# blackle/Megalania

Hardware: AMD Instinct MI355X
Metric: SA neighbour-cost evals/s (higher is better)
Workload: dtype u64

## Files before the change

megalania_amd/csrc/mgl_api.hip:

```cpp
#include "mgl_kernels.hip"
#include "mgl_kernels2.hip"
#include "mgl_kernels3.hip"
#include "mgl_kernels4.hip"
#include "mgl_kernels5.hip"
#include "mgl_pbuild.hip"
#include "mgl_index.hip"
#include "mgl_matchfinder.hip"
#include "mgl_optimal.hip"
#include "mgl_adaptive.hip"
#include "mgl_props.hip"
#include "../../include/megalania_hip.h"

#include <math.h>
#include <stdio.h>
#include <stdlib.h>
#include <string.h>
#include <string>
#include <vector>

static const uint16_t k_cost_table[2048] = {
#include "mgl_cost_table.inc"
};

#define MGL_MAX_INPUT 176000000ull
// ... 398 lines not shown
		HIPCHK(hipGetLastError());
		return MGL_OK;
	}
	if (zero_counts) HIPCHK(hipMemsetAsync(sa->d_counts, 0, 8 * sizeof(uint32_t), sa->stream));
	const uint32_t blocks2 = (K + sa->waves_per_block2 - 1) / sa->waves_per_block2;
	const bool split_now = sa->split_nbr && !sa->form_single;
	const uint32_t sim_lds_regular = ((((sa->ctx.L.total + 31u) >> 5) + 3u) & ~3u) * 4u + sa->chg_cap * 16u;
	if (split_now) {
		const uint32_t slices = nbr_slices(sa);
		HIPCHK(hipEventRecord(sa->ev_fork, sa->stream));
		if (slices >= 2) HIPCHK(hipStreamWaitEvent(sa->stream2, sa->ev_fork, 0));
		HIPCHK(hipStreamWaitEvent(sa->stream3, sa->ev_fork, 0));
		for (uint32_t h = 0; h < slices; h++) {
			const uint32_t j0 = (uint32_t)((uint64_t)K * h / slices), j1 = (uint32_t)((uint64_t)K * (h + 1) / slices);
			hipStream_t st = (h & 1u) ? sa->stream2 : sa->stream;
			hipLaunchKernelGGL((k_neighbours2<false, MGL_NBR_PICK>), dim3((j1 - j0 + sa->pick_waves - 1) / sa->pick_waves), dim3(64 * sa->pick_waves),
			                   (MGL_PICK_T_GLOBAL ? 0u : 4096u) + sa->pick_waves * sa->per_wave_pick, st, sa->ctx,
			                   sa->b2, sa->base.ctl, sa->cfg.seed, step_override, K, sa->nbr, sa->per_wave_pick, sa->d_todo, sa->d_counts,
			                   (unsigned long long*)nullptr, sa->big, sa->d_pickrec, j0, j1, sa->d_pickstate); NBR_TRACE("k_neighbours2<false, MGL_NBR_PICK>");
			hipLaunchKernelGGL((k_neighbours2<false, MGL_NBR_REST>), dim3(j1 - j0), dim3(64), sa->per_wave_rest, st, sa->ctx,
			                   sa->b2, sa->base.ctl, sa->cfg.seed, step_override, K, sa->nbr, sa->per_wave_rest, sa->d_todo, sa->d_counts,
			                   g_prof_big ? (unsigned long long*)nullptr : sa->d_prof, sa->big, sa->d_pickrec, j0, j1, sa->d_pickstate); NBR_TRACE("k_neighbours2<false, MGL_NBR_REST>");
			HIPCHK(hipEventRecord(sa->ev_rest[h], st));
		}
		HIPCHK(hipGetLastError());
		for (uint32_t h = 0; h < slices; h++) {
			const uint32_t j0 = (uint32_t)((uint64_t)K * h / slices), j1 = (uint32_t)((uint64_t)K * (h + 1) / slices);
			HIPCHK(hipStreamWaitEvent(sa->stream3, sa->ev_rest[h], 0));
			if (sa->time_sim_step >= 0 && h < 2) HIPCHK(hipEventRecord(sim_event(sa, 4 * (size_t)sa->time_sim_step + 2 * h), sa->stream3));
			if (sa->count_traffic)
				hipLaunchKernelGGL(k_sim<true>, dim3(j1 - j0), dim3(64 * sa->sim_waves), sim_lds_regular, sa->stream3, sa->ctx, sa->b2, sa->base.ctl,
				                   sa->nbr, sa->big, j0, j1, sa->d_todo3, sa->d_counts + 4, sa->d_traffic);
			else
				hipLaunchKernelGGL(k_sim<false>, dim3(j1 - j0), dim3(64 * sa->sim_waves), sim_lds_regular, sa->stream3, sa->ctx, sa->b2, sa->base.ctl,
// ... 323 lines not shown
		sa->snapshots = !(sa->cfg.flags & MGL_F_NO_SNAPSHOTS);
		if (sa->snapshots) {
			for (Base2* s : { &sa->snap_lit, &sa->snap_best }) {
				*s = b;
				s->slab = nullptr; s->onwalk = nullptr; s->sp0 = s->sp1 = s->sp2 = nullptr; s->sp_state = nullptr;
				s->ck_probs = nullptr; s->ch_off = s->ch_len = s->ch_cap = s->ch_pos = nullptr; s->ch_ev = nullptr;
				s->pool_top = nullptr;
				int rc = alloc_b2(*s, n, true, false, nullptr);
				if (rc) return rc;
			}
			HIPCHK(hipMalloc(&sa->d_snap_meta, sizeof(SnapMeta) * 2));
			HIPCHK(hipMemset(sa->d_snap_meta, 0, sizeof(SnapMeta) * 2));
			sa->d_best = sa->snap_best.slab;
		}
		if (sa->cfg.flags & MGL_F_PROFILE) {
			HIPCHK(hipMalloc(&sa->d_prof, sizeof(unsigned long long) * (32 + K)));
			HIPCHK(hipMemset(sa->d_prof, 0, sizeof(unsigned long long) * (32 + K)));
		}
		HIPCHK(hipMalloc(&sa->d_todo, sizeof(uint32_t) * (K + 1)));
		HIPCHK(hipMemset(sa->d_todo, 0, sizeof(uint32_t) * (K + 1)));
		sa->b2_bytes = bytes;
		sa->incremental_apply = getenv("MGL_NO_INCREMENTAL_APPLY") == nullptr;
		{
			ApplyBuf& ab = sa->ab;
			memset(&ab, 0, sizeof ab);
			sa->apply_blocks = 256;
			ab.scratch_cap = b.pool_cap + 256u;
			ab.span_cap = 1u << 22;
			ab.job_cap = 1u << 20;
			HIPCHK(hipMalloc(&ab.hdr, sizeof(uint32_t) * 16));
			HIPCHK(hipMemset(ab.hdr, 0, sizeof(uint32_t) * 16));
			HIPCHK(hipMalloc(&ab.ins_key, sizeof(uint16_t) * MGL_BATCH_ALLOC));
// ... 75 lines not shown
				const uint32_t tot = (160u * 1024u / bytes) * w;
				if (tot > best_total) { best_total = tot; best_w = w; }
			}
			(void)best_w;
			sa->waves_per_block2 = 1;
		}
		sa->nbr2_lds = 4096u + sa->waves_per_block2 * sa->per_wave2;
		sa->build_lds = 4096u + ckpt_elems * 2u + ckpt_elems * 8u;
		HIPCHK(hipMalloc(&sa->d_counts, sizeof(uint32_t) * 16));
		HIPCHK(hipMemset(sa->d_counts, 0, sizeof(uint32_t) * 16));
		HIPCHK(hipMalloc(&sa->d_todo3, sizeof(uint32_t) * (K + 1)));
		HIPCHK(hipMemset(sa->d_todo3, 0, sizeof(uint32_t) * (K + 1)));
		sa->big.todo_in = sa->d_todo; sa->big.todo_in_count = sa->d_counts; sa->big.spill_ctr = sa->d_counts + 2;
		HIPCHK(hipFuncSetAttribute((const void*)k_neighbours2<false, MGL_NBR_FULL>, hipFuncAttributeMaxDynamicSharedMemorySize, (int)sa->nbr2_lds));
		HIPCHK(hipFuncSetAttribute((const void*)k_neighbours2<false, MGL_NBR_PICK>, hipFuncAttributeMaxDynamicSharedMemorySize, 160 * 1024));
		HIPCHK(hipFuncSetAttribute((const void*)k_neighbours2<false, MGL_NBR_REST>, hipFuncAttributeMaxDynamicSharedMemorySize, (int)sa->nbr2_lds));
		HIPCHK(hipFuncSetAttribute((const void*)k_neighbours2<true, MGL_NBR_FULL>, hipFuncAttributeMaxDynamicSharedMemorySize, (int)(4096u + sa->per_wave2 + 12u * MGL_BIG_CAP + MGL_COOP_BYTES)));
		HIPCHK(hipMalloc(&sa->d_pickrec, sizeof(uint4) * K));
		HIPCHK(hipMalloc(&sa->d_pickstate, sizeof(uint4) * 2 * K));
		sa->split_nbr = getenv("MGL_NO_SPLIT") == nullptr;
		if (sa->split_nbr) {
			BigScratch& g = sa->big;
			HIPCHK(hipMalloc(&g.sim_hdr, sizeof(uint4) * (size_t)K));
			HIPCHK(hipMalloc(&g.sim_keys, sizeof(uint16_t) * 2u * sa->chg_cap * (size_t)K));
			HIPCHK(hipMalloc(&g.sim_pos, sizeof(uint32_t) * 2u * sa->chg_cap * (size_t)K));
			HIPCHK(hipMemset(g.sim_hdr, 0xFF, sizeof(uint4) * (size_t)K));
			if (getenv("MGL_NO_CONT") == nullptr) {
				HIPCHK(hipMalloc(&g.cont, sizeof(uint32_t) * MGL_CONT_WORDS * (size_t)g.slots));
				HIPCHK(hipMemset(g.cont, 0, sizeof(uint32_t) * MGL_CONT_WORDS * (size_t)g.slots));
			}
// ... 1208 lines not shown
	const Base2& b = sa->b2;
	const void* src = nullptr;
	size_t sz = 0;
	uint32_t top = 0;
	if (sa->incremental) HIPCHK(hipMemcpy(&top, b.pool_top, sizeof top, hipMemcpyDeviceToHost));
	switch (what) {
	case 0: src = b.ch_off; sz = sizeof(uint32_t) * sa->ctx.L.total; break;
	case 1: src = b.ch_len; sz = sizeof(uint32_t) * sa->ctx.L.total; break;
	case 2: src = b.ch_pos; sz = sizeof(uint32_t) * (size_t)top; break;
	case 3: src = b.ch_ev; sz = sizeof(uint16_t) * (size_t)top; break;
	case 4: src = b.onwalk; sz = sizeof(uint64_t) * b.nw0; break;
	case 5: src = b.sp0; sz = sizeof(uint64_t) * b.nw0; break;
	case 6: src = b.sp_state; sz = sizeof(uint32_t) * 8 * (size_t)sa->n; break;
	case 7: src = b.ck_probs; sz = sizeof(uint16_t) * (size_t)b.nck * b.ck_elems; break;
	case 8: src = b.ch_cap; sz = sizeof(uint32_t) * sa->ctx.L.total; break;
	case 9: src = sa->d_prof; sz = sa->d_prof ? sizeof(unsigned long long) * (32 + sa->cfg.neighbours_per_step) : 0; break;
	case 80: {
		const uint64_t v[3] = { sa->batch_accepts, sa->batch_fallbacks, sa->batch_early_giveups };
		*bytes = sizeof v;
		if (cap_bytes >= sizeof v) memcpy(out, v, sizeof v);
		return MGL_OK;
	}
	case 84: src = sa->lim.why; sz = sizeof(uint32_t); break;
	case 85: src = b.pool_top; sz = sizeof(uint32_t); break;
	case 83: src = b.ch_sb; sz = sizeof(uint32_t) * (size_t)b.ck_elems * b.sb_stride; break;
	case 81: src = sa->batch.hdr; sz = sizeof(uint32_t) * 16; break;
	case 82: src = sa->batch.acc; sz = sizeof(long long) * 4; break;
	case 10: src = sa->d_counts + 8; sz = sizeof(uint32_t) * 4; break;
	case 14: src = sa->ab.hdr; sz = sa->ab.hdr ? sizeof(uint32_t) * 16 : 0; break;
	case 16: src = sa->base.ctl; sz = sizeof(Control); break;
	case 15: src = sa->d_pickrec; sz = sa->d_pickrec ? sizeof(uint4) * sa->cfg.neighbours_per_step : 0; break;
// ... 76 lines not shown
```

megalania_amd/csrc/mgl_kernels.hip:

```cpp
#include "mgl_device.h"


struct TopK {
	uint64_t key;
	uint32_t count;
	uint32_t k;
};

__device__ __forceinline__ uint64_t topk_make_key(uint32_t cost, uint64_t seq)
{
	return ((uint64_t)cost << 44) | (MGL_SEQ_MASK - seq);
}
__device__ __forceinline__ uint64_t topk_threshold(const TopK& t)
{
	return t.count < t.k ? MGL_INVALID_COST : rdlane64(t.key, t.k - 1u);
}
__device__ __forceinline__ void topk_offer(TopK& t, uint64_t cand, uint32_t lane, bool allow_batch = true)
{
	const uint64_t thr0 = topk_threshold(t);
	unsigned long long m = __ballot(cand < thr0);
	if (!m) return;
	if (allow_batch && __popcll(m) >= 4) {
		uint32_t less_e = 0, less_c = 0, e_less = 0;
		for (unsigned long long mm = m; mm; mm &= mm - 1ull) {
// ... 96 lines not shown
	while (hi > lo) {
		const uint32_t span = hi - lo, step = (span + 63u) / 64u;
		const uint32_t idx = lo + lane * step;
		const bool ge = idx >= hi ? true : ((uint32_t)a[idx] >= x);
		const unsigned long long m = __ballot(ge);
		const int f = m ? __ffsll((long long)m) - 1 : 64;
		if (f == 0) break;
		const uint32_t na = lo + (uint32_t)(f - 1) * step + 1u;
		uint32_t nb = lo + (uint32_t)f * step;
		if (nb > hi) nb = hi;
		lo = na; hi = nb;
	}
	return lo;
}

template <int W>
__device__ void topk_find(TopK& t, const DevCtx& c, const Walk& w, const uint16_t* probs, const uint16_t* T,
                          uint32_t* lencost, mgl_pk incumbent, uint32_t lane)
{
	const uint32_t pos = w.st.pos;
	const uint32_t state = w.st.ctx_state;
	const uint32_t pos_state = pos & ((1u << c.L.pb) - 1u);
	const uint32_t sp = (state << 4) + pos_state;
	t.key = MGL_INVALID_COST;
	t.count = 0;
	t.k = c.top_k;

	const uint32_t c_m1 = bit_cost(probs, T, MGL_CS_IS_MATCH + sp, 1);
	const uint32_t c_r0 = bit_cost(probs, T, MGL_CS_IS_REP + state, 0);
	const uint32_t c_r1 = bit_cost(probs, T, MGL_CS_IS_REP + state, 1);
	const uint32_t g0_0 = bit_cost(probs, T, MGL_CS_G0 + state, 0), g0_1 = bit_cost(probs, T, MGL_CS_G0 + state, 1);
	const uint32_t g1_0 = bit_cost(probs, T, MGL_CS_G1 + state, 0), g1_1 = bit_cost(probs, T, MGL_CS_G1 + state, 1);
	const uint32_t g2_0 = bit_cost(probs, T, MGL_CS_G2 + state, 0), g2_1 = bit_cost(probs, T, MGL_CS_G2 + state, 1);
// ... 59 lines not shown
		uint32_t ec = 0;
		if (lane < pl.nev) {
			uint32_t ctx, bit;
			mgl_plan_event(&pl, lane, &ctx, &bit);
			ec = bit_cost(probs, T, ctx, bit);
		}
		uint32_t lit = (uint32_t)wave_sum64(ec);
		if (lane == 0 && incumbent != MGL_PK_LITERAL) cand = topk_make_key(lit, 0);
		if (lane == 1 && pos > 0 && byte == rep_byte && incumbent != MGL_PK_SHORT_REP)
			cand = topk_make_key(hdr_rep + g0_0 + l_0, 1);
		topk_offer(t, cand, lane);
	}

	if (c.diag_stop == 32) return;
	if (pos == 0 || pos >= c.n - 1) return;
	const uint32_t bigram = ((uint32_t)walk_byte_at(w, pos) << 8) | c.data[pos + 1];
	uint32_t lo = c.bucket_off[bigram];
	const uint32_t end = c.bucket_off[bigram + 1];
	const uint32_t hi = bucket_lower_bound(c.bucket_pos, lo, end, pos, lane);
	if (pos > c.dict_limit) lo = bucket_lower_bound(c.bucket_pos, lo, hi, pos - c.dict_limit, lane);
	if (c.max_scan && hi - lo > c.max_scan) lo = hi - c.max_scan;
	const uint32_t nhits = hi - lo;
	if (c.diag_stop == 33) { t.count += nhits & 1u; return; }
	if (nhits == 0) return;
	const uint32_t wpos = c.bucket_pos[lo];
	const uint32_t maxlen = (c.n - pos) < MGL_MAX_MATCH ? (c.n - pos) : MGL_MAX_MATCH;
	const uint32_t inc_type = mgl_pk_type(incumbent), inc_len = mgl_pk_len(incumbent), inc_dist = mgl_pk_dist(incumbent);

	auto price_high_lengths = [&]() {
		for (uint32_t l = 18 + lane; l <= MGL_MAX_MATCH; l += 64) {
			lencost[l - 2] = length_cost(probs, T, MGL_OFF_LEN, l, pos_state);
			lencost[272 + l - 2] = length_cost(probs, T, MGL_OFF_REP_LEN, l, pos_state);
		}
		high_ready = true;
		wave_sync();
		uint32_t a = 0xFFFFFFFFu, b = 0xFFFFFFFFu;
		for (uint32_t l = 16 + lane; l < 272; l += 64) { a = lencost[l] < a ? lencost[l] : a; b = lencost[272 + l] < b ? lencost[272 + l] : b; }
		for (int o = 32; o > 0; o >>= 1) {
			const uint32_t a2 = (uint32_t)__shfl_xor((int)a, o, 64), b2 = (uint32_t)__shfl_xor((int)b, o, 64);
			a = a2 < a ? a2 : a; b = b2 < b ? b2 : b;
		}
		minlen_m = a < minlen_m ? uni(a) : minlen_m; minlen_r = b < minlen_r ? uni(b) : minlen_r;
	};

	if (c.diag_stop == 34) return;
	{
		const uint32_t b0 = bigram >> 8, b1 = bigram & 0xFFu;
#pragma unroll
		for (uint32_t k = 0; k < 4; k++) {
			const uint32_t dk = mgl_dist_at(&w.st, k);
			if (dk >= pos) continue;
			const uint32_t q = pos - dk - 1u;
			if (q < wpos || c.data[q] != b0 || c.data[q + 1] != b1) continue;
			uint32_t L = maxlen;
			for (uint32_t base = 0; base < maxlen; base += 64) {
				const uint32_t i = base + lane;
				const bool stop = i >= maxlen || c.data[q + i] != c.data[pos + i];
				const unsigned long long m = __ballot(stop);
				if (m) { const uint32_t f = base + (uint32_t)__ffsll((long long)m) - 1u; L = f < maxlen ? f : maxlen; break; }
			}
			if (L >= 18 && !high_ready) price_high_lengths();
			const uint32_t hdr = k == 0 ? hdr_lr0 : k == 1 ? hdr_lr1 : k == 2 ? hdr_lr2 : hdr_lr3;
			for (uint32_t top = L; top >= 2;) {
				const uint64_t thr = topk_threshold(t);
				const bool nolim = thr == MGL_INVALID_COST;
				const uint32_t lim = nolim ? 0u : (uint32_t)(thr >> 44) + 1u;
				if (!nolim && hdr + minlen_r >= lim * top) break;
				uint64_t cand = MGL_INVALID_COST;
				if (lane + 2u <= top) {
					const uint32_t len = top - lane;
					const uint32_t perp = hdr + lencost[272 + len - 2];
					if ((nolim || perp < lim * len) && !(inc_type == MGL_LONG_REP && len == inc_len && inc_dist == k)) {
						const uint64_t key = topk_make_key(perp / len, ((uint64_t)(q + 1) << 12) | ((uint64_t)len << 3) | (1u + k));
						if (key < thr) cand = key;
					}
				}
				topk_offer(t, cand, lane);
				top = top > 64u + 1u ? top - 64u : 0u;
			}
		}
	}

	uint64_t x8, x16, x0;
	__builtin_memcpy(&x0, c.data + pos, 8);
	__builtin_memcpy(&x8, c.data + pos + 8, 8);
	__builtin_memcpy(&x16, c.data + pos + 16, 8);
	const uint32_t r8 = c.oct_rank[pos], r16 = c.hex_rank[pos];
	const uint32_t l8 = bucket_lower_bound(c.oct_pos, c.oct_run[r8], r8, wpos, lane);
	const uint32_t l16 = bucket_lower_bound(c.hex_pos, c.hex_run[r16], r16, wpos, lane);
	if (c.diag_stop == 35) return;
	uint32_t min15;
	{
		uint32_t m15 = lane < 14 ? lencost[lane] : 0xFFFFFFFFu;
		for (int o = 8; o > 0; o >>= 1) { const uint32_t d2 = (uint32_t)__shfl_xor((int)m15, o, 64); m15 = d2 < m15 ? d2 : m15; }
		min15 = uni(m15);
	}
	uint32_t lim32;
	{ const uint64_t th = topk_threshold(t); lim32 = th == MGL_INVALID_COST ? 0xFFFFFFFFu : (uint32_t)(th >> 44) + 1u; }
	auto price_hits = [&](uint32_t hq, uint32_t hL, bool have) {
		if (!high_ready && __ballot(have && hL >= 18)) price_high_lengths();
		const uint32_t d = pos - hq - 1u;
		uint32_t slot = d, lb = 0;
		if (have) {
			if (d >= 4) { const uint32_t nlow = mgl_msb32(d) - 2; slot = nlow * 2 + (d >> nlow); }
// ... 68 lines not shown
							__builtin_memcpy(&yy, c.data + cq + L, 8);
							const uint64_t df2 = x ^ yy;
							if (df2) { L += ((uint32_t)__ffsll((long long)df2) - 1u) >> 3; break; }
							L += 8;
						}
					}
				} else {
					const uint64_t df = x8 ^ cy;
					if (!df) have = false;
					else L = 8u + (((uint32_t)__ffsll((long long)df) - 1u) >> 3);
				}
				if (L > maxlen) L = maxlen;
			}
			price_hits(cq, L, have);
		}
	}
	if (c.diag_stop == 36 || c.diag_stop == 37) return;

	for (uint32_t D = 7; D >= 2; D--) {
		if (c.diag_stop == 38 && D < 4) break;
		const uint32_t li = D - 2u;
		const uint32_t* spos = c.xpos[li];
		const uint8_t* snxb = c.xnxb[li];
		uint32_t top, low;
		if (D == 2) { top = hi; low = lo; }
		else {
			top = c.xrank[li][pos];
			low = bucket_lower_bound(spos, c.xrun[li][top], top, wpos, lane);
		}
		const uint32_t cnt = top - low;
		if (cnt == 0) continue;
		const uint32_t xb = (uint32_t)(x0 >> (8u * D)) & 0xFFu;
		const uint32_t hitlen = D < maxlen ? D : maxlen;
		uint32_t minup;
		{
			uint32_t v = lane < D - 1u ? lencost[lane] : 0xFFFFFFFFu;
			for (int o = 4; o > 0; o >>= 1) { const uint32_t a2 = (uint32_t)__shfl_xor((int)v, o, 64); v = a2 < v ? a2 : v; }
			minup = uni(v);
		}
		uint32_t dthr = 0xFFFFFFFFu, lim_seen = 0xFFFFFFFFu;
		auto refresh_threshold = [&]() {
			lim_seen = lim32;
			dthr = 0xFFFFFFFFu;
			if (lim32 == 0xFFFFFFFFu) return;
			const uint32_t fixed = hdr_match + minup, need = lim32 * D;
// ... 16 lines not shown
			} else {
				yv = 0;
#pragma unroll
				for (uint32_t r = 0; r < (uint32_t)W; r++) {
					const bool in = e0 + r < cnt;
					const uint32_t idx = in ? top - 1u - (e0 + r) : top - 1u;
					qv[r] = in ? spos[idx] : pos;
					yv |= (uint32_t)snxb[idx] << (8u * r);
				}
			}
		};
		refresh_threshold();
		uint32_t qa[W], qb[W], ya, yb = 0;
#pragma unroll
		for (uint32_t r = 0; r < (uint32_t)W; r++) qb[r] = 0;
		loadw(0, qa, ya);
		for (uint32_t hb = 0; hb < cnt; hb += 64u * W) {
			if (hb + 64u * W < cnt) loadw(hb + 64u * W, qb, yb);
			if (lim_seen != lim32) refresh_threshold();
			if (pos - rdlane(qa[0], 0) - 1u >= dthr) break;
			uint32_t prmask = 0;
#pragma unroll
			for (uint32_t r = 0; r < (uint32_t)W; r++) {
				const uint32_t d = pos - qa[r] - 1u;
				const bool p = ((ya >> (8u * r)) & 0xFFu) != xb && d < dthr && d != 0xFFFFFFFFu;
				prmask |= (p ? 1u : 0u) << r;
			}
			if (c.diag_stop == 39) prmask = 0;
			for (uint32_t r = 0; r < (uint32_t)W && __ballot(prmask != 0); r++) {
				const bool p = (prmask >> r) & 1u;
				if (!__ballot(p)) continue;
				uint32_t q_r = qa[0];
#pragma unroll
				for (uint32_t k = 1; k < (uint32_t)W; k++) q_r = r == k ? qa[k] : q_r;
				price_hits(q_r, hitlen, p);
				prmask &= ~(1u << r);
			}
#pragma unroll
			for (uint32_t r = 0; r < (uint32_t)W; r++) qa[r] = qb[r];
			ya = yb;
		}
	}
}

__device__ __forceinline__ mgl_pk topk_packet(uint64_t key, uint32_t pos)
{
	uint64_t seq = MGL_SEQ_MASK - (key & MGL_SEQ_MASK);
	if (seq == 0) return MGL_PK_LITERAL;
	if (seq == 1) return MGL_PK_SHORT_REP;
	uint32_t q1 = (uint32_t)(seq >> 12), len = (uint32_t)(seq >> 3) & 0x1FFu, kind = (uint32_t)seq & 7u;
	if (kind == 0) return mgl_pack(MGL_MATCH, pos - q1, len);
	return mgl_pack(MGL_LONG_REP, kind - 1, len);
}


__device__ __forceinline__ void ckpt_store(const BaseView& b, const DevCtx& c, uint32_t ci, const uint16_t* probs,
// ... 115 lines not shown
};
__device__ __forceinline__ void journal_set(Journal& jn, uint32_t pos, mgl_pk old, mgl_pk neu, uint32_t lane)
{
	for (uint32_t i = 0; i < jn.count && i < 2; i++) {
		if (jn.pos[i] == pos) { if (lane == 0) jn.neu[i] = neu; wave_sync(); return; }
	}
	if (jn.count >= MGL_MAX_DIFFS) { jn.overflow = true; return; }
	if (lane == 0) { jn.pos[jn.count] = pos; jn.old[jn.count] = old; jn.neu[jn.count] = neu; }
	jn.count++;
	wave_sync();
}

struct NbrRng { uint64_t key; uint32_t n; };
__device__ __forceinline__ uint32_t nbr_draw(NbrRng& r) { return mgl_rng_draw(r.key, r.n++); }

template <int W>
__device__ bool pick_from_top_k(const DevCtx& c, const Walk& w, const uint16_t* probs, const uint16_t* T, uint32_t* lencost,
                                mgl_pk incumbent, bool best, NbrRng& rng, uint32_t lane, mgl_pk* picked)
{
	TopK t;
	topk_find<W>(t, c, w, probs, T, lencost, incumbent, lane);
	const uint32_t count = t.count;
	if (count == 0) return false;
	uint32_t choice = nbr_draw(rng) % count;
	for (int i = 0; i < 7; i++) { uint32_t x = nbr_draw(rng) % count; choice = x > choice ? x : choice; }
	if (nbr_draw(rng) % 8u == 0 || best) choice = count - 1;
	uint64_t key = shfl64(t.key, (int)(count - 1 - choice));
	*picked = topk_packet(key, w.st.pos);
	return true;
}

__device__ __forceinline__ bool long_rep_ok(const DevCtx& c, const Walk& w, uint32_t idx, uint32_t len, uint32_t lane)
{
	const uint32_t rd = mgl_dist_at(&w.st, idx);
	if (rd >= w.st.pos || w.st.pos + len > c.n) return false;
	const uint32_t src = w.st.pos - rd - 1u;
// ... 306 lines not shown
	for (uint32_t i = lane; i < 2048; i += 64) T[i] = c.cost_tbl[i];
	wave_sync();
	if (position >= c.n || !((b.onwalk[position >> 6] >> (position & 63u)) & 1ull)) {
		if (lane == 0) *out_count = ~0u;
		return;
	}
	Walk w;
	ckpt_load(b, c, position >> MGL_CKPT_SHIFT, probs, w, lane);
	while (w.st.pos < position) {
		walk_window(w, c, b.slab, lane);
		const mgl_pk pk = walk_slab_at(w, w.st.pos);
		walk_packet<true>(w, c, probs, T, mgl_pk_type(pk), mgl_pk_dist(pk), mgl_pk_len(pk), lane);
	}
	walk_window(w, c, b.slab, lane);
	TopK t;
	topk_find<4>(t, c, w, probs, T, lencost, walk_slab_at(w, position), lane);
	if (lane < t.count) {
		const uint32_t o = t.count - 1 - lane;
		out_pk[o] = topk_packet(t.key, position);
		out_cost[o] = t.key >> 44;
	}
	if (lane == 0) *out_count = t.count;
}

__global__ void k_substrings(DevCtx c, uint32_t pos, uint32_t max_len, uint32_t* offs, uint32_t* lens, uint32_t cap,
                             uint32_t* count)
{
	uint32_t k = 0;
	if (pos != 0 && pos != c.n - 1 && pos < c.n) {
		const uint32_t bg = ((uint32_t)c.data[pos] << 8) | c.data[pos + 1];
		for (uint32_t i = c.bucket_off[bg]; i < c.bucket_off[bg + 1]; i++) {
// ... 15 lines not shown
```

megalania_amd/csrc/mgl_kernels2.hip:

```cpp
#include "mgl_base2.h"


struct BitAcc {
	uint32_t word;
	uint64_t bits;
};
__device__ __forceinline__ void bitacc_move(BitAcc& a, uint64_t* arr, uint32_t new_word, uint32_t lane)
{
	if (new_word == a.word) return;
	if (lane == 0) arr[a.word] = a.bits;
	for (uint32_t z = a.word + 1 + lane; z < new_word; z += 64) arr[z] = 0;
	a.word = new_word; a.bits = 0;
}

__device__ void build_body(const DevCtx& c, const Base2& b, Control* ctl, int check_cost)
{
	extern __shared__ __attribute__((aligned(16))) unsigned char smem[];
	uint16_t* T = (uint16_t*)smem;
	uint16_t* probs = (uint16_t*)(smem + 4096);
	uint32_t* cnt = (uint32_t*)(smem + 4096 + (size_t)b.ck_elems * 2);
	uint32_t* off = cnt + b.ck_elems;
	const uint32_t lane = threadIdx.x;
	const uint32_t total = c.L.total;
	if (check_cost && !ctl->accepted_flag) return;
// ... 644 lines not shown
	return (int64_t)d;
}
__device__ __forceinline__ void coop_helpers(const DevCtx& c, const Base2& b, const BigScratch& big, unsigned long long* dbg, unsigned char* smem,
                                             uint32_t per_wave_bytes, const uint16_t* T, uint32_t lane, uint32_t wid)
{
	CoopCmd* cmd = coop_cmd(smem, per_wave_bytes);
	uint32_t seen = 0;
	for (;;) {
		__syncthreads();
		const uint32_t gen = uni(cmd->gen);
		if (uni(cmd->op) == MGL_COOP_EXIT || gen == seen) return;
		seen = gen;
		coop_share(c, b, big, dbg, smem, per_wave_bytes, T, cmd, lane, wid);
	}
}
template <bool BIG, int MODE>
__device__ __forceinline__ void nbr2_one(const DevCtx& c, const Base2& b, Control* ctl, uint64_t seed,
                                         uint64_t step_override, uint32_t K, const NbrOut& out, uint32_t per_wave_bytes,
                                         uint32_t* todo, uint32_t* todo_count, unsigned long long* prof_acc,
                                         const BigScratch& big, uint4* pickrec, uint32_t j_base, uint32_t j_end, uint4* pickstate,
                                         unsigned char* smem, const uint16_t* T, uint32_t unit, uint32_t lane, uint32_t wid)
{
	uint32_t j = j_base + unit;
	uint32_t slot = 0;
	const unsigned long long t_begin = prof_acc ? __builtin_readcyclecounter() : 0ull;
	if (BIG) {
		slot = unit;
		const uint32_t nflag = *big.todo_in_count;
		if (slot >= nflag) return;
		j = uni(big.todo_in[slot]);
		if (lane == 0) atomicAdd((unsigned long long*)&ctl->big_nbrs, 1ull);
// ... 68 lines not shown
		} else {
			rng.n = 32;
			uint32_t p = rdlane(mydraw, 31);
			uint32_t wd = p >> 6;
			uint64_t bits = b.onwalk[wd] & (~0ull << (p & 63u));
			while (!bits && ++wd < b.nw0) bits = b.onwalk[wd];
			target = uni(bits ? (wd << 6) + ctz64(bits) : 0u);
		}
		nb = uni_state(base_state_at(b, target));
		if (MODE == MGL_NBR_PICK && lane == 0) {
			pickstate[2u * j] = make_uint4(target, rng.n, nb.ctx_state, nb.dists[0]);
			pickstate[2u * j + 1u] = make_uint4(nb.dists[1], nb.dists[2], nb.dists[3], 0u);
		}
	}
	Prof prof;
	prof_start(prof, prof_acc);
	ch.dbg = prof_acc;
	ch.diag = c.diag_stop;
	const uint32_t pos = target;
	mgl_wstate bs = nb;
	Win win; win.base = 0xFFFFFFFFu; win.pk = 0; win.byte = 0;
	Walk tw;

	win_cover(win, c, b.slab, pos, lane);
	const mgl_pk first = win_pk(win, pos);
	mgl_pk m_first = first, m_second = 0;
	bool second_set = false, mutated = false;
	prof_mark(prof, 0, lane);
	if (c.diag_stop == 1) { if (lane == 0) { out.cost[j] = MGL_INVALID_COST; out.ndiffs[j] = 0; out.walked[j] = first; } return; }
	if (!(BIG && resumed) && pos + 1 < c.n && (nbr_draw(rng) % 2u) == 0) {
		const mgl_pk second = uni64(b.slab[pos + 1]);
		const uint32_t ft = mgl_pk_type(first), flen = mgl_pk_len(first);
// ... 3 lines not shown
			m_first = MGL_PK_LITERAL;
			if (MODE != MGL_NBR_PICK) { journal_set(jn, pos, first, m_first, lane); journal_set(jn, pos + 1, second, m_second, lane); }
			second_set = true; mutated = true;
		} else if ((ft == MGL_LITERAL || ft == MGL_SHORT_REP) && (st == MGL_MATCH || st == MGL_LONG_REP)) {
			uint32_t rep_start = pos - (st == MGL_LONG_REP ? mgl_dist_at(&nb, sdist) : sdist);
			if (slen < MGL_MAX_MATCH && rep_start > 0 && rep_start <= pos && win_byte(win, pos) == c.data[rep_start - 1]) {
				m_first = mgl_pack(st, sdist, slen + 1);
				if (MODE != MGL_NBR_PICK) journal_set(jn, pos, first, m_first, lane);
				mutated = true;
			}
		}
	}
	enum { P_MODEL, P_SIM, P_TOPK, P_WALK, P_OUT };
	uint32_t phase = mutated ? P_WALK : P_MODEL;
	if (MODE == MGL_NBR_PICK && mutated) return;
	if (MODE == MGL_NBR_REST && c.diag_stop != 0 && c.diag_stop != 4 && c.diag_stop < 40) return;
	bool pick_is_mutation = !mutated;
	uint32_t pick_pos = pos;
	mgl_pk pick_inc = first;
	bool pick_best = false;
	bool have_pick = false;
	mgl_pk picked_pk = 0, resume_old = 0;
	uint32_t sim_limit = MGL_POS_INF;
	bool sim_overlay = false;
	int64_t delta = 0;
	bool generate_failed = false, sim_deferred = false, walk_long = false;
	uint32_t npicks = 0;
	uint32_t count = 0;
	uint32_t walked = 0;
	uint32_t wend = 0;
// ... 42 lines not shown
				if (lane == 0) sl = atomicAdd(big.spill_ctr, 1u);
				sl = uni(sl);
				if (sl >= big.slots) { ch.overflow = true; phase = P_OUT; continue; }
				uint16_t* gik = big.ins_key + (size_t)sl * big.cap; uint32_t* gip = big.ins_pos + (size_t)sl * big.cap;
				uint16_t* grk = big.rem_key + (size_t)sl * big.cap; uint32_t* grp = big.rem_pos + (size_t)sl * big.cap;
				for (uint32_t i = lane; i < ch.n_ins; i += 64) { gik[i] = ch.ins_key[i]; gip[i] = ch.ins_pos[i]; }
				for (uint32_t i = lane; i < ch.n_rem; i += 64) { grk[i] = ch.rem_key[i]; grp[i] = ch.rem_pos[i]; }
				__threadfence_block();
				wave_sync();
				ch.ins_key = gik; ch.ins_pos = gip; ch.rem_key = grk; ch.rem_pos = grp;
				ch.uctx = big.uctx + (size_t)sl * big.uctx_cap;
				ch.cap = big.cap; ch.uctx_cap = big.uctx_cap;
				spilled = true;
			}
			model_load(c, b, probs, T, pick_pos, lane);
			if (!pick_is_mutation) prof_mark(prof, 5, lane);
			if (pick_is_mutation) {
				prof_mark(prof, 1, lane);
				if (c.diag_stop == 2) { if (lane == 0) { out.cost[j] = MGL_INVALID_COST; out.ndiffs[j] = 0; out.walked[j] = probs[lane]; } return; }
			}
			if ((ch.n_ins + ch.n_rem) != 0) { sim_limit = pick_pos; sim_overlay = true; phase = P_SIM; }
			else phase = P_TOPK;
		}
		if (MODE == MGL_NBR_REST && phase == P_SIM) {
			uint16_t* gk = big.sim_keys + (size_t)j * (2u * big.chg_cap);
			uint32_t* gp = big.sim_pos + (size_t)j * (2u * big.chg_cap);
			for (uint32_t e = lane; e < ch.n_ins; e += 64) { gk[e] = ch.ins_key[e]; gp[e] = ch.ins_pos[e]; }
			for (uint32_t e = lane; e < ch.n_rem; e += 64) { gk[big.chg_cap + e] = ch.rem_key[e]; gp[big.chg_cap + e] = ch.rem_pos[e]; }
			if (lane == 0) big.sim_hdr[j] = make_uint4(ch.n_ins, ch.n_rem, (uint32_t)(uint64_t)ch.direct, (uint32_t)((uint64_t)ch.direct >> 32));
			sim_deferred = true;
// ... 1 lines not shown
			continue;
		}
		if (MODE == MGL_NBR_FULL && phase == P_SIM) {
			int64_t r;
			if (BIG) r = coop_sim(c, b, big, prof_acc, smem, per_wave_bytes, T, ch, slot, sim_limit, sim_overlay ? probs : nullptr, lane, &too_many);
			else r = chain_sim(b, ch, T, sim_limit, sim_overlay ? probs : nullptr, lane, &too_many);
			wave_sync();
			if (too_many) { phase = P_OUT; continue; }
			if (sim_overlay) { prof_mark(prof, 6, lane); phase = P_TOPK; }
			else { delta = r; prof_mark(prof, 4, lane); phase = P_OUT; }
		}
		if (MODE != MGL_NBR_REST && phase == P_TOPK) {
			walk_from_state(tw, nb);
			walk_window(tw, c, b.slab, lane);
			mgl_pk picked;
			const bool ok = pick_from_top_k<(MODE == MGL_NBR_PICK ? 4 : 1)>(c, tw, probs, T, lencost, pick_inc, pick_best, rng, lane, &picked);
			if (MODE == MGL_NBR_PICK) {
				if (lane == 0) pickrec[j] = make_uint4((uint32_t)picked, (uint32_t)(picked >> 32), rng.n, ok ? 1u : 0u);
				return;
			}
			if (pick_is_mutation) {
				if (!ok) { generate_failed = true; phase = P_OUT; continue; }
				m_first = picked;
				journal_set(jn, pos, first, m_first, lane);
				pick_is_mutation = false;
				prof_mark(prof, 2, lane);
				if (c.diag_stop == 3 || (c.diag_stop >= 31 && c.diag_stop <= 39)) { if (lane == 0) { out.cost[j] = MGL_INVALID_COST; out.ndiffs[j] = 0; out.walked[j] = (uint32_t)m_first; } return; }
			} else {
				picked_pk = ok ? picked : pick_inc;
				have_pick = true;
				prof_mark(prof, 7, lane);
			}
			win.base = 0xFFFFFFFFu;
// ... 191 lines not shown
	for (uint32_t i = 0; i < jn.count; i++) {
		if (jn.old[i] == jn.neu[i]) continue;
		if (lane == 0) {
			out.dpos[(size_t)j * MGL_MAX_DIFFS + nd] = jn.pos[i];
			out.dold[(size_t)j * MGL_MAX_DIFFS + nd] = jn.old[i];
			out.dnew[(size_t)j * MGL_MAX_DIFFS + nd] = jn.neu[i];
		}
		nd++;
	}
	if (lane == 0) { if (!sim_deferred) out.cost[j] = total; out.ndiffs[j] = nd; out.walked[j] = walked; out.win[2u * j] = pos; out.win[2u * j + 1u] = wend; out.win2[j] = (wsoft < wend ? wsoft : wend) | (dep << 31); }
	if (prof_acc && lane == 0)
		prof_acc[32 + j] = ((__builtin_readcyclecounter() - t_begin) & 0xFFFFFFFFFFull) |
		                   ((unsigned long long)((ch.n_ins + ch.n_rem) & 0xFFFu) << 40) | ((unsigned long long)(walked & 0xFFFu) << 52);
}

template <bool BIG, int MODE>
__global__ void __launch_bounds__((MODE == MGL_NBR_PICK ? 512 : (BIG ? 64 * MGL_BIG_WAVES : 64)), (MODE == MGL_NBR_FULL ? (BIG ? 1 : MGL_NBR_WAVES_PER_SIMD) : (MODE == MGL_NBR_REST ? MGL_REST_WAVES_PER_SIMD : 4))) k_neighbours2(DevCtx c, Base2 b, Control* ctl, uint64_t seed,
                                                     uint64_t step_override, uint32_t K, NbrOut out, uint32_t per_wave_bytes,
                                                     uint32_t* todo, uint32_t* todo_count, unsigned long long* prof_acc,
                                                     BigScratch big, uint4* pickrec, uint32_t j_base, uint32_t j_end, uint4* pickstate)
{
	const uint32_t waves = blockDim.x >> 6;
	if (BIG && blockIdx.x >= *big.todo_in_count) return;
	extern __shared__ __attribute__((aligned(16))) unsigned char smem[];
	uint16_t* T = (uint16_t*)smem;
	if (BIG && threadIdx.x == 0) { CoopCmd* cmd = coop_cmd(smem, per_wave_bytes); cmd->gen = 0; cmd->op = MGL_COOP_SIM; }
	if (MODE == MGL_NBR_PICK && MGL_PICK_T_GLOBAL) {
		T = const_cast<uint16_t*>(c.cost_tbl);
	} else if (MODE != MGL_NBR_REST) {
		for (uint32_t i = threadIdx.x; i < 256; i += blockDim.x) reinterpret_cast<uint4*>(T)[i] = reinterpret_cast<const uint4*>(c.cost_tbl)[i];
		__syncthreads();
	}
	const uint32_t lane = threadIdx.x & 63u, wid = threadIdx.x >> 6;
	if (BIG) {
		if (wid != 0) { coop_helpers(c, b, big, prof_acc, smem, per_wave_bytes, T, lane, wid); return; }
		const uint32_t n = *big.todo_in_count;
		for (uint32_t unit = blockIdx.x; unit < n; unit += gridDim.x)
			nbr2_one<BIG, MODE>(c, b, ctl, seed, step_override, K, out, per_wave_bytes, todo, todo_count, prof_acc, big, pickrec, j_base, j_end, pickstate, smem, T, unit, lane, 0u);
		if (lane == 0) { CoopCmd* cmd = coop_cmd(smem, per_wave_bytes); cmd->op = MGL_COOP_EXIT; cmd->gen = cmd->gen + 1u; }
		__syncthreads();
	} else {
		nbr2_one<BIG, MODE>(c, b, ctl, seed, step_override, K, out, per_wave_bytes, todo, todo_count, prof_acc, big, pickrec, j_base, j_end, pickstate, smem, T,
		                    blockIdx.x * waves + wid, lane, wid);
	}
}


#ifndef MGL_SIM_WAVES
#define MGL_SIM_WAVES 2u
#endif
#define MGL_SIM_WAVES_MAX 8u
struct SimShared {
	uint16_t* T;
	uint32_t* dyn;
	unsigned long long* sum;
	uint32_t* nu_many;
};
// ... 114 lines not shown
```

Baseline: 14.46 million.

## Batch top-k index lookups into a per-wave plan built with lane-parallel gathers

Adds topk_plan_make, which gathers the rank, run and bucket lookups for all suffix tables and the repeat-distance match lengths in one lane-parallel pass. It then narrows every table's lower bound together with a strided ballot search, so topk_find reuses these values instead of issuing dependent serial binary searches. This is aimed at the latency of chained global loads in the pick kernel. It also adds an optional per-stage cycle profiler in a PROF template variant, selected only when profiling is enabled, and enlarges the profile buffer. The risks are more register pressure from the plan struct and extra work for tables that would otherwise be skipped.

```diff
diff --git a/megalania_amd/csrc/mgl_api.hip b/megalania_amd/csrc/mgl_api.hip
--- a/megalania_amd/csrc/mgl_api.hip
+++ b/megalania_amd/csrc/mgl_api.hip
@@ -436,10 +436,10 @@
 		for (uint32_t h = 0; h < slices; h++) {
 			const uint32_t j0 = (uint32_t)((uint64_t)K * h / slices), j1 = (uint32_t)((uint64_t)K * (h + 1) / slices);
 			hipStream_t st = (h & 1u) ? sa->stream2 : sa->stream;
-			hipLaunchKernelGGL((k_neighbours2<false, MGL_NBR_PICK>), dim3((j1 - j0 + sa->pick_waves - 1) / sa->pick_waves), dim3(64 * sa->pick_waves),
+			hipLaunchKernelGGL((sa->d_prof ? k_neighbours2<false, MGL_NBR_PICK, true> : k_neighbours2<false, MGL_NBR_PICK>), dim3((j1 - j0 + sa->pick_waves - 1) / sa->pick_waves), dim3(64 * sa->pick_waves),
 			                   (MGL_PICK_T_GLOBAL ? 0u : 4096u) + sa->pick_waves * sa->per_wave_pick, st, sa->ctx,
 			                   sa->b2, sa->base.ctl, sa->cfg.seed, step_override, K, sa->nbr, sa->per_wave_pick, sa->d_todo, sa->d_counts,
-			                   (unsigned long long*)nullptr, sa->big, sa->d_pickrec, j0, j1, sa->d_pickstate); NBR_TRACE("k_neighbours2<false, MGL_NBR_PICK>");
+			                   sa->d_prof, sa->big, sa->d_pickrec, j0, j1, sa->d_pickstate); NBR_TRACE("k_neighbours2<false, MGL_NBR_PICK>");
 			hipLaunchKernelGGL((k_neighbours2<false, MGL_NBR_REST>), dim3(j1 - j0), dim3(64), sa->per_wave_rest, st, sa->ctx,
 			                   sa->b2, sa->base.ctl, sa->cfg.seed, step_override, K, sa->nbr, sa->per_wave_rest, sa->d_todo, sa->d_counts,
 			                   g_prof_big ? (unsigned long long*)nullptr : sa->d_prof, sa->big, sa->d_pickrec, j0, j1, sa->d_pickstate); NBR_TRACE("k_neighbours2<false, MGL_NBR_REST>");
@@ -793,8 +793,8 @@
 			sa->d_best = sa->snap_best.slab;
 		}
 		if (sa->cfg.flags & MGL_F_PROFILE) {
-			HIPCHK(hipMalloc(&sa->d_prof, sizeof(unsigned long long) * (32 + K)));
-			HIPCHK(hipMemset(sa->d_prof, 0, sizeof(unsigned long long) * (32 + K)));
+			HIPCHK(hipMalloc(&sa->d_prof, sizeof(unsigned long long) * (64 + 2 * (size_t)K)));
+			HIPCHK(hipMemset(sa->d_prof, 0, sizeof(unsigned long long) * (64 + 2 * (size_t)K)));
 		}
 		HIPCHK(hipMalloc(&sa->d_todo, sizeof(uint32_t) * (K + 1)));
 		HIPCHK(hipMemset(sa->d_todo, 0, sizeof(uint32_t) * (K + 1)));
@@ -900,6 +900,7 @@
 		sa->big.todo_in = sa->d_todo; sa->big.todo_in_count = sa->d_counts; sa->big.spill_ctr = sa->d_counts + 2;
 		HIPCHK(hipFuncSetAttribute((const void*)k_neighbours2<false, MGL_NBR_FULL>, hipFuncAttributeMaxDynamicSharedMemorySize, (int)sa->nbr2_lds));
 		HIPCHK(hipFuncSetAttribute((const void*)k_neighbours2<false, MGL_NBR_PICK>, hipFuncAttributeMaxDynamicSharedMemorySize, 160 * 1024));
+		HIPCHK(hipFuncSetAttribute((const void*)k_neighbours2<false, MGL_NBR_PICK, true>, hipFuncAttributeMaxDynamicSharedMemorySize, 160 * 1024));
 		HIPCHK(hipFuncSetAttribute((const void*)k_neighbours2<false, MGL_NBR_REST>, hipFuncAttributeMaxDynamicSharedMemorySize, (int)sa->nbr2_lds));
 		HIPCHK(hipFuncSetAttribute((const void*)k_neighbours2<true, MGL_NBR_FULL>, hipFuncAttributeMaxDynamicSharedMemorySize, (int)(4096u + sa->per_wave2 + 12u * MGL_BIG_CAP + MGL_COOP_BYTES)));
 		HIPCHK(hipMalloc(&sa->d_pickrec, sizeof(uint4) * K));
@@ -2138,7 +2139,7 @@
 	case 6: src = b.sp_state; sz = sizeof(uint32_t) * 8 * (size_t)sa->n; break;
 	case 7: src = b.ck_probs; sz = sizeof(uint16_t) * (size_t)b.nck * b.ck_elems; break;
 	case 8: src = b.ch_cap; sz = sizeof(uint32_t) * sa->ctx.L.total; break;
-	case 9: src = sa->d_prof; sz = sa->d_prof ? sizeof(unsigned long long) * (32 + sa->cfg.neighbours_per_step) : 0; break;
+	case 9: src = sa->d_prof; sz = sa->d_prof ? sizeof(unsigned long long) * (64 + 2 * (size_t)sa->cfg.neighbours_per_step) : 0; break;
 	case 80: {
 		const uint64_t v[3] = { sa->batch_accepts, sa->batch_fallbacks, sa->batch_early_giveups };
 		*bytes = sizeof v;
diff --git a/megalania_amd/csrc/mgl_kernels.hip b/megalania_amd/csrc/mgl_kernels.hip
--- a/megalania_amd/csrc/mgl_kernels.hip
+++ b/megalania_amd/csrc/mgl_kernels.hip
@@ -134,9 +134,128 @@
 	return lo;
 }
 
-template <int W>
+#define MGL_PICK_STAGES 16u
+struct PickProf {
+	unsigned long long* acc;
+	unsigned long long t;
+};
+__device__ __forceinline__ void pick_prof_mark(PickProf* p, uint32_t stage, uint32_t lane)
+{
+	if (!p || !p->acc) return;
+	const unsigned long long now = __builtin_readcyclecounter();
+	if (lane == 0) { atomicAdd(&p->acc[stage], now - p->t); atomicAdd(&p->acc[MGL_PICK_STAGES + stage], 1ull); }
+	p->t = __builtin_readcyclecounter();
+}
+
+#ifndef MGL_PICK_BATCH
+#define MGL_PICK_BATCH 1
+#endif
+struct TopkPlan {
+	uint32_t lo, hi;
+	uint32_t wmin;
+	uint32_t r16, l16, r8, l8;
+	uint32_t top[5], low[5];
+	uint32_t rep;
+	uint64_t x0, x8, x16;
+};
+__device__ __forceinline__ void topk_plan_make(TopkPlan& p, const DevCtx& c, const mgl_wstate& st, uint32_t lane)
+{
+	const uint32_t pos = st.pos;
+	p.lo = p.hi = p.wmin = p.r16 = p.l16 = p.r8 = p.l8 = p.rep = 0;
+#pragma unroll
+	for (uint32_t i = 0; i < 5; i++) p.top[i] = p.low[i] = 0;
+	p.x0 = p.x8 = p.x16 = 0;
+	if (pos == 0 || pos >= c.n - 1) return;
+	const uint32_t maxlen = (c.n - pos) < MGL_MAX_MATCH ? (c.n - pos) : MGL_MAX_MATCH;
+	const uint32_t* rt = lane == 0 ? c.oct_rank : lane == 1 ? c.hex_rank : lane == 2 ? c.xrank[1] : lane == 3 ? c.xrank[2] :
+	                     lane == 4 ? c.xrank[3] : lane == 5 ? c.xrank[4] : c.xrank[5];
+	uint32_t rk = 0;
+	if (lane < 7) rk = rt[pos];
+	uint64_t xw = 0;
+	if (lane < 3) __builtin_memcpy(&xw, c.data + pos + 8u * lane, 8);
+	const uint32_t pv = c.data[pos + lane];
+	uint32_t qv[4];
+#pragma unroll
+	for (uint32_t k = 0; k < 4; k++) {
+		const uint32_t dk = mgl_dist_at(&st, k);
+		qv[k] = dk < pos ? (uint32_t)c.data[pos - dk - 1u + lane] : 0x100u;
+	}
+#pragma unroll
+	for (uint32_t k = 0; k < 4; k++) {
+		if (mgl_dist_at(&st, k) >= pos) continue;
+		const unsigned long long m = __ballot(lane >= maxlen || qv[k] != pv);
+		p.rep |= (m ? (uint32_t)__ffsll((long long)m) - 1u : 64u) << (8u * k);
+	}
+	p.x0 = rdlane64(xw, 0); p.x8 = rdlane64(xw, 1); p.x16 = rdlane64(xw, 2);
+	p.r8 = rdlane(rk, 0); p.r16 = rdlane(rk, 1);
+#pragma unroll
+	for (uint32_t i = 0; i < 5; i++) p.top[i] = rdlane(rk, 2u + i);
+	const uint32_t bigram = (((uint32_t)p.x0 & 0xFFu) << 8) | (((uint32_t)p.x0 >> 8) & 0xFFu);
+	const uint32_t* st1 = lane < 2 ? c.bucket_off : lane == 2 ? c.oct_run : lane == 3 ? c.hex_run : lane == 4 ? c.xrun[1] :
+	                      lane == 5 ? c.xrun[2] : lane == 6 ? c.xrun[3] : lane == 7 ? c.xrun[4] : c.xrun[5];
+	const uint32_t i1 = lane < 2 ? bigram + lane : lane == 2 ? p.r8 : lane == 3 ? p.r16 : lane == 4 ? p.top[0] :
+	                    lane == 5 ? p.top[1] : lane == 6 ? p.top[2] : lane == 7 ? p.top[3] : p.top[4];
+	uint32_t s1 = 0;
+	if (lane < 9) s1 = st1[i1];
+	const uint32_t off0 = rdlane(s1, 0), off1 = rdlane(s1, 1);
+	const uint32_t floor = pos > c.dict_limit ? pos - c.dict_limit : 0u;
+	const uint32_t* const tab[9] = { c.bucket_pos, c.bucket_pos, c.oct_pos, c.hex_pos, c.xpos[1], c.xpos[2], c.xpos[3], c.xpos[4], c.xpos[5] };
+	uint32_t a[9], b[9];
+	a[0] = a[1] = off0; b[0] = b[1] = off1;
+	a[2] = rdlane(s1, 2); b[2] = p.r8;
+	a[3] = rdlane(s1, 3); b[3] = p.r16;
+#pragma unroll
+	for (uint32_t i = 0; i < 5; i++) { a[4u + i] = rdlane(s1, 4u + i); b[4u + i] = p.top[i]; }
+	const bool capped = c.max_scan != 0;
+	uint32_t xlow = floor;
+	uint32_t on = capped ? 0x003u : (floor != 0 ? 0x1FFu : 0x001u);
+	if (floor == 0) on &= ~2u;
+#pragma nounroll
+	for (uint32_t pass = 0; pass < 2; pass++) {
+		if (pass == 1) {
+			if (!capped) break;
+			p.hi = a[0]; p.lo = floor != 0 ? a[1] : off0;
+			if (p.hi - p.lo > c.max_scan) p.lo = p.hi - c.max_scan;
+			if (p.hi == p.lo) return;
+			xlow = uni(c.bucket_pos[p.lo]);
+			on = 0x1FCu;
+		}
+		for (;;) {
+			uint32_t v[9];
+			bool any = false;
+#pragma unroll
+			for (uint32_t s = 0; s < 9; s++) {
+				v[s] = 0xFFFFFFFFu;
+				if (!((on >> s) & 1u) || b[s] <= a[s]) continue;
+				any = true;
+				const uint32_t idx = a[s] + lane * ((b[s] - a[s] + 63u) / 64u);
+				if (idx < b[s]) v[s] = tab[s][idx];
+			}
+			if (!any) break;
+#pragma unroll
+			for (uint32_t s = 0; s < 9; s++) {
+				if (!((on >> s) & 1u) || b[s] <= a[s]) continue;
+				const uint32_t step = (b[s] - a[s] + 63u) / 64u;
+				const unsigned long long m = __ballot(v[s] >= (s == 0 ? pos : xlow));
+				const int f = m ? __ffsll((long long)m) - 1 : 64;
+				if (f == 0) { b[s] = a[s]; continue; }
+				const uint32_t na = a[s] + (uint32_t)(f - 1) * step + 1u;
+				uint32_t nb = a[s] + (uint32_t)f * step;
+				if (nb > b[s]) nb = b[s];
+				a[s] = na; b[s] = nb;
+			}
+		}
+	}
+	if (!capped) { p.hi = a[0]; p.lo = floor != 0 ? a[1] : off0; }
+	p.wmin = xlow;
+	p.l8 = a[2]; p.l16 = a[3];
+#pragma unroll
+	for (uint32_t i = 0; i < 5; i++) p.low[i] = a[4u + i];
+}
+
+template <int W, bool BATCH = false, bool PROF = false>
 __device__ void topk_find(TopK& t, const DevCtx& c, const Walk& w, const uint16_t* probs, const uint16_t* T,
-                          uint32_t* lencost, mgl_pk incumbent, uint32_t lane)
+                          uint32_t* lencost, mgl_pk incumbent, uint32_t lane, const TopkPlan* plan = nullptr, PickProf* pp = nullptr)
 {
 	const uint32_t pos = w.st.pos;
 	const uint32_t state = w.st.ctx_state;
@@ -226,16 +345,22 @@
 
 	if (c.diag_stop == 32) return;
 	if (pos == 0 || pos >= c.n - 1) return;
-	const uint32_t bigram = ((uint32_t)walk_byte_at(w, pos) << 8) | c.data[pos + 1];
-	uint32_t lo = c.bucket_off[bigram];
-	const uint32_t end = c.bucket_off[bigram + 1];
-	const uint32_t hi = bucket_lower_bound(c.bucket_pos, lo, end, pos, lane);
-	if (pos > c.dict_limit) lo = bucket_lower_bound(c.bucket_pos, lo, hi, pos - c.dict_limit, lane);
-	if (c.max_scan && hi - lo > c.max_scan) lo = hi - c.max_scan;
+	if (PROF) pick_prof_mark(pp, 3, lane);
+	uint32_t lo, hi, bigram = 0;
+	if (BATCH) { lo = plan->lo; hi = plan->hi; }
+	else {
+		bigram = ((uint32_t)walk_byte_at(w, pos) << 8) | c.data[pos + 1];
+		lo = c.bucket_off[bigram];
+		const uint32_t end = c.bucket_off[bigram + 1];
+		hi = bucket_lower_bound(c.bucket_pos, lo, end, pos, lane);
+		if (pos > c.dict_limit) lo = bucket_lower_bound(c.bucket_pos, lo, hi, pos - c.dict_limit, lane);
+		if (c.max_scan && hi - lo > c.max_scan) lo = hi - c.max_scan;
+	}
 	const uint32_t nhits = hi - lo;
 	if (c.diag_stop == 33) { t.count += nhits & 1u; return; }
 	if (nhits == 0) return;
-	const uint32_t wpos = c.bucket_pos[lo];
+	const uint32_t wpos = BATCH ? plan->wmin : c.bucket_pos[lo];
+	if (PROF) pick_prof_mark(pp, 4, lane);
 	const uint32_t maxlen = (c.n - pos) < MGL_MAX_MATCH ? (c.n - pos) : MGL_MAX_MATCH;
 	const uint32_t inc_type = mgl_pk_type(incumbent), inc_len = mgl_pk_len(incumbent), inc_dist = mgl_pk_dist(incumbent);
 
@@ -263,9 +388,10 @@
 			const uint32_t dk = mgl_dist_at(&w.st, k);
 			if (dk >= pos) continue;
 			const uint32_t q = pos - dk - 1u;
-			if (q < wpos || c.data[q] != b0 || c.data[q + 1] != b1) continue;
-			uint32_t L = maxlen;
-			for (uint32_t base = 0; base < maxlen; base += 64) {
+			const uint32_t L0 = BATCH ? (plan->rep >> (8u * k)) & 0xFFu : 0u;
+			if (BATCH ? (q < wpos || L0 < 2u) : (q < wpos || c.data[q] != b0 || c.data[q + 1] != b1)) continue;
+			uint32_t L = (BATCH && L0 < 64u) ? L0 : maxlen;
+			for (uint32_t base = BATCH ? (L0 < 64u ? maxlen : 64u) : 0u; base < maxlen; base += 64) {
 				const uint32_t i = base + lane;
 				const bool stop = i >= maxlen || c.data[q + i] != c.data[pos + i];
 				const unsigned long long m = __ballot(stop);
@@ -293,13 +419,19 @@
 		}
 	}
 
+	if (PROF) pick_prof_mark(pp, 5, lane);
 	uint64_t x8, x16, x0;
-	__builtin_memcpy(&x0, c.data + pos, 8);
-	__builtin_memcpy(&x8, c.data + pos + 8, 8);
-	__builtin_memcpy(&x16, c.data + pos + 16, 8);
-	const uint32_t r8 = c.oct_rank[pos], r16 = c.hex_rank[pos];
-	const uint32_t l8 = bucket_lower_bound(c.oct_pos, c.oct_run[r8], r8, wpos, lane);
-	const uint32_t l16 = bucket_lower_bound(c.hex_pos, c.hex_run[r16], r16, wpos, lane);
+	uint32_t r8, r16, l8, l16;
+	if (BATCH) { x0 = plan->x0; x8 = plan->x8; x16 = plan->x16; r8 = plan->r8; r16 = plan->r16; l8 = plan->l8; l16 = plan->l16; }
+	else {
+		__builtin_memcpy(&x0, c.data + pos, 8);
+		__builtin_memcpy(&x8, c.data + pos + 8, 8);
+		__builtin_memcpy(&x16, c.data + pos + 16, 8);
+		r8 = c.oct_rank[pos]; r16 = c.hex_rank[pos];
+		l8 = bucket_lower_bound(c.oct_pos, c.oct_run[r8], r8, wpos, lane);
+		l16 = bucket_lower_bound(c.hex_pos, c.hex_run[r16], r16, wpos, lane);
+	}
+	if (PROF) pick_prof_mark(pp, 4, lane);
 	if (c.diag_stop == 35) return;
 	uint32_t min15;
 	{
@@ -398,6 +530,7 @@
 			}
 			price_hits(cq, L, have);
 		}
+		if (PROF) pick_prof_mark(pp, 6 + ph, lane);
 	}
 	if (c.diag_stop == 36 || c.diag_stop == 37) return;
 
@@ -408,11 +541,15 @@
 		const uint8_t* snxb = c.xnxb[li];
 		uint32_t top, low;
 		if (D == 2) { top = hi; low = lo; }
-		else {
+		else if (BATCH) {
+			top = D == 7 ? plan->top[4] : D == 6 ? plan->top[3] : D == 5 ? plan->top[2] : D == 4 ? plan->top[1] : plan->top[0];
+			low = D == 7 ? plan->low[4] : D == 6 ? plan->low[3] : D == 5 ? plan->low[2] : D == 4 ? plan->low[1] : plan->low[0];
+		} else {
 			top = c.xrank[li][pos];
 			low = bucket_lower_bound(spos, c.xrun[li][top], top, wpos, lane);
 		}
 		const uint32_t cnt = top - low;
+		if (PROF && cnt == 0) pick_prof_mark(pp, 4, lane);
 		if (cnt == 0) continue;
 		const uint32_t xb = (uint32_t)(x0 >> (8u * D)) & 0xFFu;
 		const uint32_t hitlen = D < maxlen ? D : maxlen;
@@ -459,6 +596,7 @@
 		uint32_t qa[W], qb[W], ya, yb = 0;
 #pragma unroll
 		for (uint32_t r = 0; r < (uint32_t)W; r++) qb[r] = 0;
+		if (PROF) pick_prof_mark(pp, 4, lane);
 		loadw(0, qa, ya);
 		for (uint32_t hb = 0; hb < cnt; hb += 64u * W) {
 			if (hb + 64u * W < cnt) loadw(hb + 64u * W, qb, yb);
@@ -485,6 +623,7 @@
 			for (uint32_t r = 0; r < (uint32_t)W; r++) qa[r] = qb[r];
 			ya = yb;
 		}
+		if (PROF) pick_prof_mark(pp, 6u + (9u - D), lane);
 	}
 }
 
@@ -630,12 +769,13 @@
 struct NbrRng { uint64_t key; uint32_t n; };
 __device__ __forceinline__ uint32_t nbr_draw(NbrRng& r) { return mgl_rng_draw(r.key, r.n++); }
 
-template <int W>
+template <int W, bool BATCH = false, bool PROF = false>
 __device__ bool pick_from_top_k(const DevCtx& c, const Walk& w, const uint16_t* probs, const uint16_t* T, uint32_t* lencost,
-                                mgl_pk incumbent, bool best, NbrRng& rng, uint32_t lane, mgl_pk* picked)
+                                mgl_pk incumbent, bool best, NbrRng& rng, uint32_t lane, mgl_pk* picked,
+                                const TopkPlan* plan = nullptr, PickProf* pp = nullptr)
 {
 	TopK t;
-	topk_find<W>(t, c, w, probs, T, lencost, incumbent, lane);
+	topk_find<W, BATCH, PROF>(t, c, w, probs, T, lencost, incumbent, lane, plan, pp);
 	const uint32_t count = t.count;
 	if (count == 0) return false;
 	uint32_t choice = nbr_draw(rng) % count;
@@ -972,7 +1112,9 @@
 	}
 	walk_window(w, c, b.slab, lane);
 	TopK t;
-	topk_find<4>(t, c, w, probs, T, lencost, walk_slab_at(w, position), lane);
+	TopkPlan plan;
+	if (MGL_PICK_BATCH) topk_plan_make(plan, c, w.st, lane);
+	topk_find<4, MGL_PICK_BATCH != 0>(t, c, w, probs, T, lencost, walk_slab_at(w, position), lane, &plan);
 	if (lane < t.count) {
 		const uint32_t o = t.count - 1 - lane;
 		out_pk[o] = topk_packet(t.key, position);
diff --git a/megalania_amd/csrc/mgl_kernels2.hip b/megalania_amd/csrc/mgl_kernels2.hip
--- a/megalania_amd/csrc/mgl_kernels2.hip
+++ b/megalania_amd/csrc/mgl_kernels2.hip
@@ -682,7 +682,7 @@
 		coop_share(c, b, big, dbg, smem, per_wave_bytes, T, cmd, lane, wid);
 	}
 }
-template <bool BIG, int MODE>
+template <bool BIG, int MODE, bool PROF = false>
 __device__ __forceinline__ void nbr2_one(const DevCtx& c, const Base2& b, Control* ctl, uint64_t seed,
                                          uint64_t step_override, uint32_t K, const NbrOut& out, uint32_t per_wave_bytes,
                                          uint32_t* todo, uint32_t* todo_count, unsigned long long* prof_acc,
@@ -781,8 +781,11 @@
 		}
 	}
 	Prof prof;
-	prof_start(prof, prof_acc);
-	ch.dbg = prof_acc;
+	prof_start(prof, MODE == MGL_NBR_PICK ? nullptr : prof_acc);
+	ch.dbg = MODE == MGL_NBR_PICK ? nullptr : prof_acc;
+	PickProf pp;
+	pp.acc = PROF ? prof_acc + 32u + K : nullptr;
+	pp.t = t_begin;
 	ch.diag = c.diag_stop;
 	const uint32_t pos = target;
 	mgl_wstate bs = nb;
@@ -816,6 +819,12 @@
 	enum { P_MODEL, P_SIM, P_TOPK, P_WALK, P_OUT };
 	uint32_t phase = mutated ? P_WALK : P_MODEL;
 	if (MODE == MGL_NBR_PICK && mutated) return;
+	TopkPlan plan;
+	if (MODE == MGL_NBR_PICK) {
+		if (PROF) pick_prof_mark(&pp, 0, lane);
+		if (MGL_PICK_BATCH) topk_plan_make(plan, c, nb, lane);
+		if (PROF) pick_prof_mark(&pp, 1, lane);
+	}
 	if (MODE == MGL_NBR_REST && c.diag_stop != 0 && c.diag_stop != 4 && c.diag_stop < 40) return;
 	bool pick_is_mutation = !mutated;
 	uint32_t pick_pos = pos;
@@ -888,6 +897,7 @@
 				spilled = true;
 			}
 			model_load(c, b, probs, T, pick_pos, lane);
+			if (PROF) pick_prof_mark(&pp, 2, lane);
 			if (!pick_is_mutation) prof_mark(prof, 5, lane);
 			if (pick_is_mutation) {
 				prof_mark(prof, 1, lane);
@@ -919,9 +929,13 @@
 			walk_from_state(tw, nb);
 			walk_window(tw, c, b.slab, lane);
 			mgl_pk picked;
-			const bool ok = pick_from_top_k<(MODE == MGL_NBR_PICK ? 4 : 1)>(c, tw, probs, T, lencost, pick_inc, pick_best, rng, lane, &picked);
+			bool ok;
+			if constexpr (MODE == MGL_NBR_PICK) ok = pick_from_top_k<4, MGL_PICK_BATCH != 0, PROF>(c, tw, probs, T, lencost, pick_inc, pick_best, rng, lane, &picked, &plan, &pp);
+			else ok = pick_from_top_k<1>(c, tw, probs, T, lencost, pick_inc, pick_best, rng, lane, &picked);
 			if (MODE == MGL_NBR_PICK) {
 				if (lane == 0) pickrec[j] = make_uint4((uint32_t)picked, (uint32_t)(picked >> 32), rng.n, ok ? 1u : 0u);
+				if (PROF) pick_prof_mark(&pp, 14, lane);
+				if (PROF && pp.acc && lane == 0) pp.acc[2u * MGL_PICK_STAGES + j] = __builtin_readcyclecounter() - t_begin;
 				return;
 			}
 			if (pick_is_mutation) {
@@ -1143,7 +1157,7 @@
 		                   ((unsigned long long)((ch.n_ins + ch.n_rem) & 0xFFFu) << 40) | ((unsigned long long)(walked & 0xFFFu) << 52);
 }
 
-template <bool BIG, int MODE>
+template <bool BIG, int MODE, bool PROF = false>
 __global__ void __launch_bounds__((MODE == MGL_NBR_PICK ? 512 : (BIG ? 64 * MGL_BIG_WAVES : 64)), (MODE == MGL_NBR_FULL ? (BIG ? 1 : MGL_NBR_WAVES_PER_SIMD) : (MODE == MGL_NBR_REST ? MGL_REST_WAVES_PER_SIMD : 4))) k_neighbours2(DevCtx c, Base2 b, Control* ctl, uint64_t seed,
                                                      uint64_t step_override, uint32_t K, NbrOut out, uint32_t per_wave_bytes,
                                                      uint32_t* todo, uint32_t* todo_count, unsigned long long* prof_acc,
@@ -1165,11 +1179,11 @@
 		if (wid != 0) { coop_helpers(c, b, big, prof_acc, smem, per_wave_bytes, T, lane, wid); return; }
 		const uint32_t n = *big.todo_in_count;
 		for (uint32_t unit = blockIdx.x; unit < n; unit += gridDim.x)
-			nbr2_one<BIG, MODE>(c, b, ctl, seed, step_override, K, out, per_wave_bytes, todo, todo_count, prof_acc, big, pickrec, j_base, j_end, pickstate, smem, T, unit, lane, 0u);
+			nbr2_one<BIG, MODE, PROF>(c, b, ctl, seed, step_override, K, out, per_wave_bytes, todo, todo_count, prof_acc, big, pickrec, j_base, j_end, pickstate, smem, T, unit, lane, 0u);
 		if (lane == 0) { CoopCmd* cmd = coop_cmd(smem, per_wave_bytes); cmd->op = MGL_COOP_EXIT; cmd->gen = cmd->gen + 1u; }
 		__syncthreads();
 	} else {
-		nbr2_one<BIG, MODE>(c, b, ctl, seed, step_override, K, out, per_wave_bytes, todo, todo_count, prof_acc, big, pickrec, j_base, j_end, pickstate, smem, T,
+		nbr2_one<BIG, MODE, PROF>(c, b, ctl, seed, step_override, K, out, per_wave_bytes, todo, todo_count, prof_acc, big, pickrec, j_base, j_end, pickstate, smem, T,
 		                    blockIdx.x * waves + wid, lane, wid);
 	}
 }
```

Result: faster. 14.79 million, median of 6 (+2.2%).
